# Grice-Lab/HmmUFOtu

Measured on AMD Instinct MI355X. Metric: reads placed/sec (whole node), gg_97_otus GTR+dGamma 250bp; HBM GB/s %peak, higher is better.
Workload: dtype f64; 1 GPU; gg_97_otus-scale synthetic DB (198643 nodes x 7682 CS columns, K=1400), GTR+dGamma(4), SE 250 bp amplicon reads, batch 8192 reads/step/GPU, 6 batches in flight, seeds in the reference's std::sort order (k_seed_refsort); seed_order=reference, message_window_cols=7682, parallelism=read-sharded x1

## Files before the change

### hmmufotu_amd/csrc/hu_engine.hip

```cpp
#include <algorithm>
#include <cmath>
#include <cstdio>
#include <cstring>
#include <limits>
#include <map>
#include <atomic>
#include <thread>
#include <memory>
#include <mutex>
#include <chrono>
#include <fstream>
#include <sstream>
#include <new>
#include <stdexcept>
#include "hu_common.h"
#include "hu_kern_sep.h"
#include "hu_kern_align.h"
#include "hu_kern_tree.h"
#include "hu_kern_blk.h"
#include "hu_kern_refsort.h"
#include "hu_kern_rank.h"
#include "hu_kern_anneal.h"
#include "hu_kern_build.h"
#include "hu_kern_otucs.h"
// ... 2267 lines not shown
		HIPCHK(hu_wait(b->stream));
	}
	b->seedCap = 1;
	for(size_t r = 0; r < n; ++r) b->seedCap = std::max(b->seedCap, (int) n_seeds[r]);
	b->state = ST_SEEDED;
	return HU_OK;
} catch(...) { return hu_catch_all("hu_seed_batch_given"); }

__global__ void k_seed_sortkeys(int n, const int32_t* __restrict__ seedCnt, const int32_t* __restrict__ seedId, uint32_t* __restrict__ key, uint32_t* __restrict__ val) {
	const int i = blockIdx.x * 256 + threadIdx.x;
	if(i >= n * HU_MAX_SEEDS) return;
	key[i] = (i % HU_MAX_SEEDS) < seedCnt[i / HU_MAX_SEEDS] ? (uint32_t) seedId[i] : 0xffffffffu;
	val[i] = (uint32_t) i;
}

static void plan_width_split(hu_batch* b) {
	b->rMain = 0; b->wideReads.clear(); b->maxAll = b->maxMain = 1;
	if((int) b->hStart.size() < b->n || (int) b->hEnd.size() < b->n) return;
	std::vector<int> R((size_t) b->n);
	for(int r = 0; r < b->n; ++r) { R[r] = std::max(0, b->hEnd[r] - b->hStart[r] + 1); b->maxAll = std::max(b->maxAll, R[r]); }
	b->maxMain = b->maxAll;
	if(!b->knob.width_split || b->n < 256) return;
	const int W = std::min(64, b->n / 128);
	std::vector<int> tmp(R);
	std::nth_element(tmp.begin(), tmp.begin() + W, tmp.end(), std::greater<int>());
	const int kth = tmp[W];
	static const int bounds[] = {512, 768, 1024, 1536, 2048, 3072};
	int bound = 0;
	for(int x : bounds) if(kth <= x) { bound = x; break; }
	if(!bound || bound >= b->maxAll) return;
	b->rMain = bound; b->maxMain = 1;
	for(int r = 0; r < b->n; ++r) { if(R[r] > bound) b->wideReads.push_back(r); else b->maxMain = std::max(b->maxMain, R[r]); }
	if(b->knob.trace) fprintf(stderr, "[hu] width split: %zu of %d reads beyond %d columns (widest %d) take a launch of their own\n", b->wideReads.size(), b->n, bound, b->maxAll);
}
static HuDbDev width_pass_dev(const hu_batch* b, int pass, const uint32_t* wideList) {
	HuDbDev dev = b->db->dev;
	if(b->rMain) { dev.rLo = pass ? b->rMain : -1; dev.rHi = pass ? 0x7fffffff : b->rMain; dev.wideList = pass ? wideList : nullptr; }
	return dev;
}

extern "C" int hu_estimate_batch(hu_batch* b, const hu_opts* o) try {
	if(!b || !o) return HU_ERR_ARG;
	if(b->state < ST_SEEDED) { hu_set_error("hu_estimate_batch: no seeds"); return HU_ERR_STATE; }
	HIPCHK(hipSetDevice(b->db->device));
	const size_t n = (size_t) b->n;
	int rc;
	if((rc = b->dEst.ensure(n * HU_MAX_SEEDS)) != HU_OK) return rc;
	(void) hipGetLastError();
	if(n) {
		Timer t(b, HU_T_ESTIMATE);
		plan_width_split(b);
		const bool stream = b->knob.streaming_sep != 0;
		if(b->rMain) {
			b->hWideOrd.clear();
			for(int r : b->wideReads) for(int sd = 0; sd < HU_MAX_SEEDS; ++sd) b->hWideOrd.push_back((uint32_t) r * HU_MAX_SEEDS + sd);
			if((rc = b->dWideOrd.ensure(b->hWideOrd.size())) != HU_OK) return rc;
			HIPCHK(hipMemcpyAsync(b->dWideOrd.p, b->hWideOrd.data(), b->hWideOrd.size() * 4, hipMemcpyHostToDevice, b->stream));
		}
		for(int pass = 0; pass < (b->rMain ? 2 : 1); ++pass) {
			const int maxR = pass ? b->maxAll : b->maxMain;
			const HuDbDev dev = width_pass_dev(b, pass, b->dWideOrd.p);
			#define EST_ARGS dev, b->db->mdl, b->dCodes.p, b->dStart.p, b->dEnd.p, b->dParDN.p, b->dSeedCnt.p, b->dSeedId.p, b->dSeedDN.p, o->weighted, b->dEst.p
			const unsigned eg = pass ? (unsigned) b->hWideOrd.size() : (unsigned) b->n * HU_MAX_SEEDS;
			const uint32_t* order = nullptr;
			if(pass) order = b->dWideOrd.p;
			else if(!b->knob.est_unsorted) {
				if((rc = b->dSortK.ensure((size_t) eg * 2)) != HU_OK || (rc = b->dSortV.ensure((size_t) eg * 2)) != HU_OK) return rc;
				k_seed_sortkeys<<<(eg + 255) / 256, 256, 0, b->stream>>>(b->n, b->dSeedCnt.p, b->dSeedId.p, b->dSortK.p, b->dSortV.p);
				if((rc = order_by_key(b, b->dSortK.p, b->dSortV.p, (size_t) eg, (uint32_t) b->db->dev.nNodes, b->dSortV.p + eg, false)) != HU_OK) return rc;
				order = b->dSortV.p + eg;
			}
			const int spt = (maxR + 255) / 256;
			const int xm = b->knob.xcd_map;
			const unsigned egl = pass ? eg : order ? std::min<unsigned>(eg, (unsigned) b->n * (unsigned) b->seedCap) : eg;
			const int var = b->knob.est_var;
			if(stream || spt > 12) k_estimate<<<eg, 64, 0, b->stream>>>(EST_ARGS);
			else if(var == 2) {
				if(spt <= 2) k_estimate_blk<2, 256><<<eg, 256, 0, b->stream>>>(EST_ARGS);
				else if(spt <= 4) k_estimate_blk<4, 256><<<eg, 256, 0, b->stream>>>(EST_ARGS);
				else if(spt <= 6) k_estimate_blk<6, 256><<<eg, 256, 0, b->stream>>>(EST_ARGS);
				else if(spt <= 8) k_estimate_blk<8, 256><<<eg, 256, 0, b->stream>>>(EST_ARGS);
				else k_estimate_blk<12, 256><<<eg, 256, 0, b->stream>>>(EST_ARGS);
			}
			else if(var == 1 && spt <= 6) k_estimate_prod<12, 2><<<egl, 128, 0, b->stream>>>(EST_ARGS, order, xm);
			else if(var == 3 && spt <= 6) k_estimate_prod<6, 4, 1><<<egl, 256, 0, b->stream>>>(EST_ARGS, order, xm);
			else if(spt <= 2) k_estimate_prod<2, 4><<<egl, 256, 0, b->stream>>>(EST_ARGS, order, xm);
			else if(spt <= 4) k_estimate_prod<4, 4><<<egl, 256, 0, b->stream>>>(EST_ARGS, order, xm);
			else if(spt <= 6) k_estimate_prod<6, 4, 4><<<egl, 256, (size_t)(b->knob.est_lds_pad > 0 && b->knob.est_lds_pad <= 60 ? b->knob.est_lds_pad : 0) * 1024, b->stream>>>(EST_ARGS, order, xm);
			else if(spt <= 8) k_estimate_prod<8, 4><<<egl, 256, 0, b->stream>>>(EST_ARGS, order, xm);
			else if(var == 4) k_estimate_prod<12, 4><<<egl, 256, 0, b->stream>>>(EST_ARGS, order, xm);
			else k_estimate_prod<6, 8, 2><<<egl, 512, 0, b->stream>>>(EST_ARGS, order, xm);
			#undef EST_ARGS
		}
	}
	HIPCHK(hipGetLastError());
	if(n) {
		if((rc = b->dPermCnt.ensure(n * 2)) != HU_OK) return rc;
		k_site_count<<<b->n, 64, 0, b->stream>>>(b->db->dev, b->n, b->dCodes.p, b->dStart.p, b->dEnd.p, b->dPermCnt.p);
		HIPCHK(hipGetLastError());
	}
	b->state = ST_ESTIMATED;
	return HU_OK;
} catch(...) { return hu_catch_all("hu_estimate_batch"); }


static int sync_host_cands(hu_batch* b) {
	if(b->hostCands) return HU_OK;
	const size_t n = (size_t) b->n;
	std::vector<int32_t> off(n + 1, 0);
	b->places.resize(b->nc);
	HIPCHK(hipSetDevice(b->db->device));
	if(n) HIPCHK(hipMemcpyAsync(off.data(), b->dCandOff.p, (n + 1) * 4, hipMemcpyDeviceToHost, b->stream));
	if(b->nc) HIPCHK(hipMemcpyAsync(b->places.data(), b->dPlaces.p, b->nc * sizeof(HuPlaceRec), hipMemcpyDeviceToHost, b->stream));
	HIPCHK(hu_wait(b->stream));
	b->candOffs.assign(off.begin(), off.end());
	b->hostCands = true;
	return HU_OK;
}
static int scan_cands(hu_batch* b, bool withPerm) {
	int rc;
	if((rc = b->dCandOff.ensure((size_t) b->n + 1)) != HU_OK || (rc = b->dMeta.ensure(4)) != HU_OK) return rc;
	k_cand_scan<<<1, 1024, 0, b->stream>>>(b->n, b->dCandCnt.p, b->dCandOff.p, withPerm ? b->dPermCnt.p : nullptr, b->dStart.p, b->dEnd.p, b->dMeta.p, b->rMain);
	HIPCHK(hipGetLastError());
	b->hMeta.assign(4, 0);
	int32_t* meta = b->hMeta.data();
	HIPCHK(hipMemcpyAsync(meta, b->dMeta.p, 12, hipMemcpyDeviceToHost, b->stream));
	if(b->rMain) { b->hCandOffAll.resize((size_t) b->n + 1); HIPCHK(hipMemcpyAsync(b->hCandOffAll.data(), b->dCandOff.p, ((size_t) b->n + 1) * 4, hipMemcpyDeviceToHost, b->stream)); }
	HIPCHK(hu_wait(b->stream));
	b->nc = (size_t) meta[0]; b->maxGapSites = meta[1]; b->maxBaseSites = meta[2];
	return HU_OK;
}

extern "C" int hu_filter_batch(hu_batch* b, const hu_opts* o) try {
	if(!b || !o) return HU_ERR_ARG;
	if(b->state < ST_ESTIMATED) { hu_set_error("hu_filter_batch: no estimates"); return HU_ERR_STATE; }
	if(!(o->max_error >= 0)) { hu_set_error("max_error must be >= 0"); return HU_ERR_ARG; }
	HIPCHK(hipSetDevice(b->db->device));
	const size_t n = (size_t) b->n;
	if(b->knob.inject_fault == 1) parallel_for(std::max<size_t>(n, 600), [&](size_t r) { if(r + 1 == std::max<size_t>(n, 600)) throw std::bad_alloc(); });
	int rc;
	if((rc = b->dCandCnt.ensure(std::max<size_t>(n, 1))) != HU_OK || (rc = b->dFiltSlot.ensure(std::max<size_t>(n, 1) * HU_MAX_SEEDS)) != HU_OK) return rc;
	(void) hipGetLastError();
	b->nc = 0; b->maxGapSites = b->maxBaseSites = 0;
	if(n) {
		k_filter<<<(unsigned)((n + 3) / 4), 256, 0, b->stream>>>(b->n, b->dSeedCnt.p, b->dEst.p, o->max_error, b->dCandCnt.p, b->dFiltSlot.p, b->knob.sort_seq);
		HIPCHK(hipGetLastError());
		if((rc = scan_cands(b, true)) != HU_OK) return rc;
		if((rc = b->dCands.ensure(std::max<size_t>(b->nc, 1))) != HU_OK || (rc = b->dPlaces.ensure(std::max<size_t>(b->nc, 1))) != HU_OK) return rc;
		k_build_cands<<<(unsigned)((n * HU_MAX_SEEDS + 255) / 256), 256, 0, b->stream>>>(b->db->dev, b->n, b->dCandCnt.p, b->dCandOff.p, b->dFiltSlot.p, b->dSeedId.p, b->dEst.p, b->dCands.p, b->dPlaces.p);
		HIPCHK(hipGetLastError());
	}
	b->hostCands = false; b->placesGiven = false;
	b->state = ST_FILTERED;
	return HU_OK;
} catch(...) { return hu_catch_all("hu_filter_batch"); }

extern "C" int hu_batch_set_candidates(hu_batch* b, const int64_t* offs, const hu_place_rec* recs, int placed) try {
	if(!b || !offs) { hu_set_error("hu_batch_set_candidates: null argument"); return HU_ERR_ARG; }
	if(b->state < ST_ALIGNED) { hu_set_error("hu_batch_set_candidates: reads are not aligned"); return HU_ERR_STATE; }
	const hu_db* db = b->db;
	const size_t n = (size_t) b->n;
	if(offs[0] != 0) { hu_set_error("hu_batch_set_candidates: offs[0] must be 0"); return HU_ERR_ARG; }
	for(size_t r = 0; r < n; ++r) {
		const int64_t k = offs[r + 1] - offs[r];
		if(k < 0 || k > HU_MAX_SEEDS || (k > 0 && (!recs || b->hAlns[r].status != HU_READ_OK || b->hEnd[r] < b->hStart[r]))) {
			hu_set_error("hu_batch_set_candidates: read %zu: %lld candidates (0..%d, none for a read that is not placed)", r, (long long) k, HU_MAX_SEEDS); return HU_ERR_ARG;
// ... 23 lines not shown
	}
	{
		int rc;
		if((rc = b->dCandCnt.ensure(std::max<size_t>(n, 1))) != HU_OK || (rc = b->dCands.ensure(std::max<size_t>(nc, 1))) != HU_OK ||
				(rc = b->dPlaces.ensure(std::max<size_t>(nc, 1))) != HU_OK || (rc = b->dPermCnt.ensure(std::max<size_t>(n, 1) * 2)) != HU_OK) return rc;
		(void) hipGetLastError();
		if(n) {
			HIPCHK(hipMemcpyAsync(b->dCandCnt.p, hCnt.data(), n * 4, hipMemcpyHostToDevice, b->stream));
			if(nc) {
				HIPCHK(hipMemcpyAsync(b->dCands.p, b->hCands.data(), nc * sizeof(HuCand), hipMemcpyHostToDevice, b->stream));
				HIPCHK(hipMemcpyAsync(b->dPlaces.p, b->places.data(), nc * sizeof(HuPlaceRec), hipMemcpyHostToDevice, b->stream));
			}
			k_site_count<<<b->n, 64, 0, b->stream>>>(db->dev, b->n, b->dCodes.p, b->dStart.p, b->dEnd.p, b->dPermCnt.p);
			HIPCHK(hipGetLastError());
			plan_width_split(b);
			if((rc = scan_cands(b, true)) != HU_OK) return rc;
		}
		else { b->nc = 0; b->maxGapSites = b->maxBaseSites = 0; }
	}
	b->hostCands = true;
	b->placesGiven = placed != 0;
	b->fixedRoot = false;
	b->state = placed ? ST_PLACED : ST_FILTERED;
	return HU_OK;
} catch(...) { return hu_catch_all("hu_batch_set_candidates"); }

__global__ void k_cand_sortkeys(int nc, const HuCand* __restrict__ cands, uint32_t* __restrict__ key, uint32_t* __restrict__ val) {
	const int i = blockIdx.x * 256 + threadIdx.x;
	if(i >= nc) return;
	key[i] = (uint32_t) cands[i].node; val[i] = (uint32_t) i;
}

extern "C" int hu_place_batch(hu_batch* b, const hu_opts* o) try {
	if(!b || !o) return HU_ERR_ARG;
	if(b->state < ST_FILTERED) { hu_set_error("hu_place_batch: candidates are not filtered"); return HU_ERR_STATE; }
	HIPCHK(hipSetDevice(b->db->device));
	const size_t nc = b->nc;
	int rc;
	if((rc = b->dPlaceOut.ensure(std::max<size_t>(nc, 1))) != HU_OK) return rc;
	(void) hipGetLastError();
	if(nc) {
		Timer t(b, HU_T_PLACE);
		int passes = 1;
		if(b->rMain) {
			b->hWideCand.clear();
			if(b->hCandOffAll.size() < (size_t) b->n + 1) { hu_set_error("hu_place_batch: candidate offsets of the wide reads are missing"); return HU_ERR_STATE; }
			for(int r : b->wideReads) for(int32_t c = b->hCandOffAll[r]; c < b->hCandOffAll[r + 1]; ++c) b->hWideCand.push_back((uint32_t) c);
			if(!b->hWideCand.empty()) {
				if((rc = b->dWideCand.ensure(b->hWideCand.size())) != HU_OK) return rc;
				HIPCHK(hipMemcpyAsync(b->dWideCand.p, b->hWideCand.data(), b->hWideCand.size() * 4, hipMemcpyHostToDevice, b->stream));
				passes = 2;
			}
		}
		for(int pass = 0; pass < passes; ++pass) {
			const int maxR = pass ? b->maxAll : b->maxMain;
			const HuDbDev dev = width_pass_dev(b, pass, b->dWideCand.p);
			const unsigned grid = pass ? (unsigned) b->hWideCand.size() : (unsigned) nc;
			const int spt2 = (maxR + 127) / 128, spt4 = (maxR + 255) / 256;
			const bool stream = b->knob.streaming_sep != 0 || spt4 > 12;
			#define PL_ARGS dev, b->db->mdl, b->dCodes.p, b->dStart.p, b->dEnd.p, b->dCands.p, b->dPlaceOut.p
			if(stream) {
				const size_t lds = (size_t)(3 * HU_MAX_DGK * 4 + HU_MAX_DGK * 5 * 4 + maxR) * sizeof(double);
				if(lds > 160 * 1024) { hu_set_error("alignment region of %d columns does not fit the placement kernel's LDS", maxR); return HU_ERR_ARG; }
				if(lds > 64 * 1024) HIPCHK(hipFuncSetAttribute((const void*) k_place, hipFuncAttributeMaxDynamicSharedMemorySize, (int) lds));
				k_place<<<grid, 64, lds, b->stream>>>(PL_ARGS);
			}
			else {
				const int var = b->knob.place_var;
				const int xm = b->knob.xcd_map;
				const uint32_t* order = nullptr;
				if(pass) order = b->dWideCand.p;
				else if(!b->knob.place_unsorted) {
					if((rc = b->dSortK.ensure(nc * 2)) != HU_OK || (rc = b->dSortV.ensure(nc * 2)) != HU_OK) return rc;
					k_cand_sortkeys<<<(unsigned)((nc + 255) / 256), 256, 0, b->stream>>>((int) nc, b->dCands.p, b->dSortK.p, b->dSortV.p);
					if((rc = order_by_key(b, b->dSortK.p, b->dSortV.p, nc, (uint32_t) b->db->dev.nNodes, b->dSortV.p + nc, false)) != HU_OK) return rc;
					order = b->dSortV.p + nc;
				}
				#define PL_GO(S, NW, E, R, O) k_place_blk<S, NW, E, R, O><<<grid, 64 * NW, 0, b->stream>>>(PL_ARGS, nullptr, order, nullptr, nullptr, xm)
				if((var == 99 || var == 98) && spt4 <= 6) {
					DBuf<long long> ddb;
					if((rc = ddb.ensure(nc * 12)) != HU_OK) return rc;
					long long* dd = ddb.p;
					HIPCHK(hipMemsetAsync(dd, 0, nc * 12 * sizeof(long long), b->stream));
					if(var == 99) k_place_blk<6, 4, 3, 0, 1, true><<<grid, 256, 0, b->stream>>>(PL_ARGS, dd);
					else k_place_blk<12, 2, 3, 0, 2, true, 1><<<grid, 128, 0, b->stream>>>(PL_ARGS, dd);
					std::vector<long long> hd(nc * 12);
					HIPCHK(hipMemcpyAsync(hd.data(), dd, nc * 12 * sizeof(long long), hipMemcpyDeviceToHost, b->stream));
					HIPCHK(hu_wait(b->stream));
					double acc[8] = {0}, ae[4] = {0};
					for(size_t c = 0; c < nc; ++c) { for(int i = 0; i < 8; ++i) acc[i] += (double) hd[c * 8 + i]; for(int i = 0; i < 4; ++i) ae[i] += (double) hd[nc * 8 + c * 4 + i]; }
					fprintf(stderr, "[place dbg] per candidate (s_memtime ticks): load %.0f tables %.0f sweeps %.0f em %.0f total %.0f | outer %.2f em steps %.2f\n",
							acc[0] / nc, acc[1] / nc, acc[2] / nc, acc[3] / nc, acc[4] / nc, acc[5] / nc, acc[6] / nc);
					fprintf(stderr, "[place dbg] inside the EM steps, per step: arithmetic %.0f wave reduction %.0f exchange between the waves %.0f tail %.0f\n",
							ae[0] / acc[6], ae[1] / acc[6], ae[2] / acc[6], ae[3] / acc[6]);
				}
				else if(var == 4 && spt4 <= 6) PL_GO(6, 4, 1, 0, 1);
				else if(var == 5 && spt4 <= 6) PL_GO(6, 4, 2, 1, 1);
				else if(var == 6 && spt2 <= 12) PL_GO(12, 2, 1, 0, 2);
				else if(spt2 <= 4) PL_GO(4, 2, 3, 0, 2);
				else if(spt2 <= 12 && !(var == 7)) {
					const int S = spt2 <= 8 ? 8 : 12, G = S - 2;
					const bool split = !pass && !b->knob.place_nosplit && b->maxGapSites <= G * 128 && b->maxBaseSites <= (S - G) * 128;
					if(b->knob.trace) fprintf(stderr, "[hu] place: %zu candidates, max region %d, %d sites per thread, %s, %s\n", nc, maxR, S, split ? "gap/base split slots" : "column order", "EM across both waves");
					if(split) {
						if((rc = b->dPerm.ensure((size_t) b->n * S * 128)) != HU_OK) return rc;
						k_site_perm<<<b->n, 64, 0, b->stream>>>(dev, b->n, b->dCodes.p, b->dStart.p, b->dEnd.p, G * 128, (S - G) * 128, b->dPerm.p);
						if(S == 8 && var != 6) k_place_blk<8, 2, 3, 0, 3, false, 3, 6><<<grid, 128, 3 * 8 * 128 * sizeof(double), b->stream>>>(PL_ARGS, nullptr, order, b->dPerm.p, b->dPermCnt.p, xm);
						else if(S == 8) k_place_blk<8, 2, 3, 0, 2, false, 0, 6><<<grid, 128, 0, b->stream>>>(PL_ARGS, nullptr, order, b->dPerm.p, b->dPermCnt.p, xm);
						else k_place_blk<12, 2, 3, 0, 2, false, 1, 10><<<grid, 128, (size_t)(b->knob.place_lds_pad > 0 && b->knob.place_lds_pad <= 44 ? b->knob.place_lds_pad : 0) * 1024, b->stream>>>(PL_ARGS, nullptr, order, b->dPerm.p, b->dPermCnt.p, xm);
					}
					else if(S == 8) PL_GO(8, 2, 3, 0, 2);
					else k_place_blk<12, 2, 3, 0, 2, false, 1><<<grid, 128, 0, b->stream>>>(PL_ARGS, nullptr, order, nullptr, nullptr, xm);
				}
				else if(var == 7 && spt2 <= 12) PL_GO(12, 2, 3, 0, 2);
				else if(spt4 <= 8) PL_GO(8, 4, 3, 0, 1);
				else if(var == 9) PL_GO(12, 4, 3, 0, 1);
				else k_place_blk<12, 4, 3, 0, 2, false, 1><<<grid, 256, 0, b->stream>>>(PL_ARGS, nullptr, order, nullptr, nullptr, xm);
				#undef PL_GO
			}
			#undef PL_ARGS
		}
		HIPCHK(hipGetLastError());
		if(o->fix_root_loglik) {
			if((rc = b->dRootLL.ensure(nc)) != HU_OK) return rc;
			k_root_loglik<<<(unsigned) nc, 64, 0, b->stream>>>(b->db->dev, b->db->mdl, b->dCodes.p, b->dStart.p, b->dEnd.p, b->dCands.p, b->dPlaceOut.p, (int) nc, b->dRootLL.p);
			HIPCHK(hipGetLastError());
		}
	}
	b->fixedRoot = o->fix_root_loglik != 0 && nc > 0;
	b->placesGiven = false;
	b->state = ST_PLACED;
	return HU_OK;
} catch(...) { return hu_catch_all("hu_place_batch"); }


static int hu_alleq_table(int device) {
	static std::mutex mu; static bool done[64] = {false};
	std::lock_guard<std::mutex> lk(mu);
	if(device < 0 || device >= 64) { hu_set_error("device %d out of range", device); return HU_ERR_ARG; }
	if(done[device]) return HU_OK;
	(void) hipGetLastError();
	k_alleq_init<<<1, 128>>>();
	HIPCHK(hipGetLastError());
	HIPCHK(hipDeviceSynchronize());
	done[device] = true;
	return HU_OK;
}

extern "C" int hu_finish_batch(hu_batch* b, const hu_opts* o) try {
	if(!b || !o) return HU_ERR_ARG;
	if(b->state < ST_PLACED) { hu_set_error("hu_finish_batch: candidates are not placed"); return HU_ERR_STATE; }
	const hu_db* db = b->db;
	const size_t n = (size_t) b->n;
	if(b->knob.inject_fault == 2) throw std::length_error("injected");
	HIPCHK(hipSetDevice(db->device));
	b->best.assign(n, hu_place_rec());
	int rc;
	if((rc = b->dBest.ensure(std::max<size_t>(n, 1))) != HU_OK) return rc;
	(void) hipGetLastError();
	if(n) {
		if((rc = hu_alleq_table(db->device)) != HU_OK) return rc;
		k_finish<<<(unsigned)((n + 63) / 64), 64, 0, b->stream>>>(db->dev, b->n, b->dStart.p, b->dEnd.p, b->dCandOff.p, b->dPlaces.p, b->dPlaceOut.p,
				b->fixedRoot ? b->dRootLL.p : nullptr, db->dLlTab, db->dAnnoId, o->max_height, o->only_ml, o->prior, b->placesGiven ? 1 : 0, b->dBest.p, b->knob.sort_seq);
		HIPCHK(hipGetLastError());
		HIPCHK(hipMemcpyAsync(b->best.data(), b->dBest.p, n * sizeof(hu_place_rec), hipMemcpyDeviceToHost, b->stream));
		HIPCHK(hu_wait(b->stream));
	}
	b->hostCands = false;
	b->state = ST_FINISHED;
	return HU_OK;
} catch(...) { return hu_catch_all("hu_finish_batch"); }

extern "C" int hu_assign_batch(hu_batch* b, const hu_opts* o) try {
	int rc;
// ... 807 lines not shown
```

### hmmufotu_amd/csrc/hu_kern_blk.h

```cpp
#pragma once
#include "hu_kern_sep.h"

#define HU_BLK_THREADS 256

__device__ inline void lds_wave_sync() { asm volatile("s_waitcnt lgkmcnt(0)" ::: "memory"); }
__device__ inline void lds_barrier() { asm volatile("s_waitcnt lgkmcnt(0)\n\ts_barrier" ::: "memory"); }

template<int NW = 4>
__device__ inline double block_sum(double v, double* red, int& phase) {
	v = wave_sum_uniform(v);
	double* r = red + (phase & 1) * NW;
	if((threadIdx.x & 63) == 0) r[threadIdx.x >> 6] = v;
	lds_barrier();
	double s = r[0];
#pragma unroll
	for(int w = 1; w < NW; ++w) s += r[w];
	phase ^= 1;
	return s;
}
template<int NW = 4>
__device__ inline long long block_sum_ll(long long v, long long* red, int& phase) {
	for(int m = 32; m > 0; m >>= 1) v += __shfl_xor(v, m);
	long long* r = red + (phase & 1) * NW;
	if((threadIdx.x & 63) == 0) r[threadIdx.x >> 6] = v;
// ... 43 lines not shown
			const int j = tid + THREADS * t;
			const int jj = j < n ? j : 0;
			load4(db.up + (sOff + jj) * 4, eU[t]); load4(db.down + (sOff + jj) * 4, eV[t]);
			bb[t] = cd[jj];
			if(j < n) ksum += (long long) db.upK[sOff + jj] + (long long) db.downK[sOff + jj];
		}
#pragma unroll
		for(int t = 0; t < SPT; ++t) {
			double c[4];
			conv_eig(mdl, Eu, eU[t], z[t]);
			conv_eig(mdl, Ev, eV[t], c);
			for(int i = 0; i < 4; ++i) z[t][i] *= c[i];
		}
	}
	int phase = 0;
	double dsum = 0, nsum = 0;
#pragma unroll
	for(int t = 0; t < SPT; ++t) {
		if(tid + THREADS * t >= n) continue;
		const int b = bb[t];
		const int b1 = argmax4_tied_lin(z[t]), b2 = b >= 0 ? b : piMax;
		if(!weighted) { if(b1 != b2) dsum += 1; }
		else {
			const double w1 = sel4(z[t], b1) / ((z[t][0] + z[t][2]) + (z[t][1] + z[t][3]));
			const double w2 = b >= 0 ? 1.0 : piw[b2];
			if(b1 != b2) dsum += w1 * w2;
			nsum += w1 * w2;
		}
	}
	dsum = block_sum<NW>(dsum, red, phase);
	double wnr;
	if(!weighted) wnr = dsum / (double) n;
	else { nsum = block_sum<NW>(nsum, red, phase); wnr = dsum / nsum; }
	double En[4], Ppi[4];
#pragma unroll
	for(int k = 0; k < 4; ++k) En[k] = exp(mdl.lam[k] * wnr);
	{ double a[4]; to_eig(mdl, mdl.pi, a); if(wnr == 0) { for(int i = 0; i < 4; ++i) Ppi[i] = mdl.pi[i]; } else conv_eig(mdl, En, a, Ppi); }
	double ll = 0;
#pragma unroll
	for(int t = 0; t < SPT; ++t) {
		if(tid + THREADS * t >= n) continue;
		const int b = bb[t];
		double c[4];
		if(b >= 0) {
			if(wnr == 0) { for(int i = 0; i < 4; ++i) c[i] = i == b ? 1.0 : 0.0; }
			else { double a[4]; for(int k = 0; k < 4; ++k) a[k] = mdl.U1[k*4+b]; conv_eig(mdl, En, a, c); }
		}
		else for(int i = 0; i < 4; ++i) c[i] = Ppi[i];
		ll += log((mdl.pi[0] * z[t][0] * c[0] + mdl.pi[2] * z[t][2] * c[2]) + (mdl.pi[1] * z[t][1] * c[1] + mdl.pi[3] * z[t][3] * c[3]));
	}
	ll = block_sum<NW>(ll, red, phase);
	int lphase = 0;
	const long long kt = block_sum_ll<NW>(ksum, redl, lphase);
	ll += (double) kt * HU_LN2;
	if(tid == 0) { HuEstOut o; o.ratio = ratio; o.wnr = wnr; o.loglik = ll; out[(size_t) read * HU_MAX_SEEDS + s] = o; }
}

template<int CTRL>
__device__ inline double dpp_mul_full(double v) {
	const int lo = __builtin_amdgcn_mov_dpp(__double2loint(v), CTRL, 0xf, 0xf, true);
	const int hi = __builtin_amdgcn_mov_dpp(__double2hiint(v), CTRL, 0xf, 0xf, true);
	return v * __hiloint2double(hi, lo);
}
__device__ inline double wave_prod(double v) {
	v = dpp_mul_full<0xB1>(v);
	v = dpp_mul_full<0x4E>(v);
	v = dpp_mul_full<0x141>(v);
	v = dpp_mul_full<0x140>(v);
	v *= __shfl_xor(v, 16);
	v *= __shfl_xor(v, 32);
	return v;
}
__device__ inline int wave_sum_i32(int v) {
	for(int m = 32; m > 0; m >>= 1) v += __shfl_xor(v, m);
	return v;
}

__device__ inline uint32_t hu_xcd_pos(uint32_t b, uint32_t nb, int xmap) {
	if(!xmap) return b;
	const uint32_t per = nb >> 3;
	return b < per * 8 ? (b & 7u) * per + (b >> 3) : b;
}

template<int SPT, int NW, int OCC = 1>
__global__ __launch_bounds__(64 * NW, OCC) void k_estimate_prod(HuDbDev db, HuModelDev mdl, const int8_t* __restrict__ codes,
		const int32_t* __restrict__ rstart, const int32_t* __restrict__ rend, const uint32_t* __restrict__ parDN,
		const int32_t* __restrict__ seedCnt, const int32_t* __restrict__ seedId, const uint32_t* __restrict__ seedDN,
		int weighted, HuEstOut* __restrict__ out, const uint32_t* __restrict__ order, int xmap = 0) {
	constexpr int THREADS = 64 * NW;
	__shared__ double redd[2 * NW];
	__shared__ int redi[2 * NW];
	__shared__ __attribute__((aligned(16))) double Qtab[NW][24];
	const uint32_t slot = order ? order[hu_xcd_pos(blockIdx.x, gridDim.x, xmap)] : blockIdx.x;
	const int read = slot / HU_MAX_SEEDS, s = slot % HU_MAX_SEEDS, tid = threadIdx.x, lane = tid & 63, wave = tid >> 6;
	if(s >= seedCnt[read] || hu_skip_width(db, rend[read] - rstart[read] + 1)) return;
	const int un = seedId[(size_t) read * HU_MAX_SEEDS + s];
	const int vn = db.parent[un];
	const uint32_t dn = seedDN[(size_t) read * HU_MAX_SEEDS + s];
	const uint32_t pv = parDN[(size_t) read * HU_MAX_SEEDS + s];
	const double cDist = (double)(dn >> 16) / (double)(dn & 0xffffu);
	const double pDist = (double)(pv >> 16) / (double)(pv & 0xffffu);
	double ratio = cDist / (cDist + pDist);
	if(isnan(ratio)) ratio = 0.5;
	const double w0 = db.blen[un];
	const double wur = w0 * ratio, wvr = w0 - wur;
	double Eu[3], Ev[3];
	{
		const int l6 = lane < 6 ? lane : 0, m3 = l6 % 3;
		const double e = exp((m3 == 0 ? mdl.lam[1] : m3 == 1 ? mdl.lam[2] : mdl.lam[3]) * (l6 < 3 ? wur : wvr));
		const int lo = __double2loint(e), hi = __double2hiint(e);
#pragma unroll
		for(int k = 0; k < 3; ++k) {
			Eu[k] = __hiloint2double(__builtin_amdgcn_readlane(hi, k), __builtin_amdgcn_readlane(lo, k));
			Ev[k] = __hiloint2double(__builtin_amdgcn_readlane(hi, 3 + k), __builtin_amdgcn_readlane(lo, 3 + k));
		}
	}
	const int start = rstart[read], end = rend[read], n = end - start + 1;
	const int8_t* __restrict__ cd = codes + (size_t) read * db.csLen + start;
	const int64_t sOff = (int64_t) un * db.winLen + (start - db.winStart);
	const int piMax = argmax4d(mdl.logpi);
	double z[SPT][4]; unsigned long long bop = 0; int ksum = 0;
	{
		double aU[SPT][4], aV[SPT][4];
#pragma unroll
		for(int t = 0; t < SPT; ++t) {
			const int j = tid + THREADS * t;
			const int jj = j < n ? j : 0;
			load4(db.up + (sOff + jj) * 4, aU[t]); load4(db.down + (sOff + jj) * 4, aV[t]);
			const int b = cd[jj];
			bop |= (unsigned long long)(b >= 0 ? b : 4) << (3 * t);
			if(j < n) ksum += db.upK[sOff + jj] + db.downK[sOff + jj];
		}
#pragma unroll
		for(int t = 0; t < SPT; ++t) {
			const double su1 = Eu[0] * aU[t][1], su2 = Eu[1] * aU[t][2], su3 = Eu[2] * aU[t][3];
			const double sv1 = Ev[0] * aV[t][1], sv2 = Ev[1] * aV[t][2], sv3 = Ev[2] * aV[t][3];
#pragma unroll
			for(int i = 0; i < 4; ++i) {
				const double cu = fmax(fma(mdl.U[i*4+3], su3, fma(mdl.U[i*4+2], su2, fma(mdl.U[i*4+1], su1, aU[t][0]))), 0.0);
				const double cv = fmax(fma(mdl.U[i*4+3], sv3, fma(mdl.U[i*4+2], sv2, fma(mdl.U[i*4+1], sv1, aV[t][0]))), 0.0);
				z[t][i] = cu * cv;
			}
		}
	}
	double wnr;
	if(!weighted) {
		int nd = 0;
#pragma unroll
		for(int t = 0; t < SPT; ++t) {
			const int bi = (int)((bop >> (3 * t)) & 7u);
			const int b1 = argmax4_tied_lin(z[t]), b2 = bi < 4 ? bi : piMax;
			nd += __popcll(__ballot(tid + THREADS * t < n && b1 != b2));
		}
		if(lane == 0) redi[wave] = nd;
		lds_barrier();
		int tot = redi[0];
#pragma unroll
		for(int w = 1; w < NW; ++w) tot += redi[w];
		wnr = (double) tot / (double) n;
	}
	else {
		double piw[4];
		{ double mx = max4d(mdl.logpi), sm; for(int i = 0; i < 4; ++i) piw[i] = exp(mdl.logpi[i] - mx); sm = (piw[0] + piw[2]) + (piw[1] + piw[3]); for(int i = 0; i < 4; ++i) piw[i] /= sm; }
		double dsum = 0, nsum = 0;
#pragma unroll
		for(int t = 0; t < SPT; ++t) {
			if(tid + THREADS * t >= n) continue;
			const int bi = (int)((bop >> (3 * t)) & 7u);
			const int b1 = argmax4_tied_lin(z[t]), b2 = bi < 4 ? bi : piMax;
			const double w1 = sel4(z[t], b1) / ((z[t][0] + z[t][2]) + (z[t][1] + z[t][3]));
			const double w2 = bi < 4 ? 1.0 : piw[b2];
			if(b1 != b2) dsum += w1 * w2;
			nsum += w1 * w2;
		}
		dsum = wave_sum(dsum); nsum = wave_sum(nsum);
		if(lane == 0) { redd[wave] = dsum; redd[NW + wave] = nsum; }
		lds_barrier();
		double a = redd[0], c = redd[NW];
#pragma unroll
		for(int w = 1; w < NW; ++w) { a += redd[w]; c += redd[NW + w]; }
		wnr = a / c;
		lds_barrier();
	}
	double* Q = Qtab[wave];
	if(lane < 3) Q[1 + lane] = exp((lane == 0 ? mdl.lam[1] : lane == 1 ? mdl.lam[2] : mdl.lam[3]) * wnr);
	lds_wave_sync();
	if(lane < 20) {
		const int b = lane >> 2, i = lane & 3;
		const double pii = sel4(mdl.pi, i);
		double c;
		if(wnr == 0) c = b < 4 ? (i == b ? 1.0 : 0.0) : pii;
		else {
			double a0, a1, a2, a3;
			if(b < 4) { a0 = sel4(mdl.U1 + 0, b); a1 = sel4(mdl.U1 + 4, b); a2 = sel4(mdl.U1 + 8, b); a3 = sel4(mdl.U1 + 12, b); }
			else {
				a0 = (mdl.U1[0] * mdl.pi[0] + mdl.U1[1] * mdl.pi[1]) + (mdl.U1[2] * mdl.pi[2] + mdl.U1[3] * mdl.pi[3]);
				a1 = (mdl.U1[4] * mdl.pi[0] + mdl.U1[5] * mdl.pi[1]) + (mdl.U1[6] * mdl.pi[2] + mdl.U1[7] * mdl.pi[3]);
				a2 = (mdl.U1[8] * mdl.pi[0] + mdl.U1[9] * mdl.pi[1]) + (mdl.U1[10] * mdl.pi[2] + mdl.U1[11] * mdl.pi[3]);
				a3 = (mdl.U1[12] * mdl.pi[0] + mdl.U1[13] * mdl.pi[1]) + (mdl.U1[14] * mdl.pi[2] + mdl.U1[15] * mdl.pi[3]);
			}
			const double Ui1 = i == 0 ? mdl.U[1] : i == 1 ? mdl.U[5] : i == 2 ? mdl.U[9] : mdl.U[13];
			const double Ui2 = i == 0 ? mdl.U[2] : i == 1 ? mdl.U[6] : i == 2 ? mdl.U[10] : mdl.U[14];
			const double Ui3 = i == 0 ? mdl.U[3] : i == 1 ? mdl.U[7] : i == 2 ? mdl.U[11] : mdl.U[15];
			c = fmax(fma(Ui3, Q[3] * a3, fma(Ui2, Q[2] * a2, fma(Ui1, Q[1] * a1, a0))), 0.0);
		}
		Q[4 + b * 4 + i] = pii * c;
	}
	lds_wave_sync();
	double mant = 1.0; int esum = ksum;
#pragma unroll
	for(int t = 0; t < SPT; ++t) {
		const double* q = Q + 4 + ((bop >> (3 * t)) & 7u) * 4;
		double x = fmax(fma(q[3], z[t][3], fma(q[2], z[t][2], fma(q[1], z[t][1], q[0] * z[t][0]))), 0.0);
		if(tid + THREADS * t >= n) x = 1.0;
		mant *= __builtin_amdgcn_frexp_mant(x);
		esum += x == 0.0 ? 0 : __builtin_amdgcn_frexp_exp(x);
	}
	esum += __builtin_amdgcn_frexp_exp(mant); mant = __builtin_amdgcn_frexp_mant(mant);
	mant = wave_prod(mant);
	esum = wave_sum_i32(esum);
	if(lane == 0) { redd[wave] = mant; redi[NW + wave] = esum; }
	lds_barrier();
	if(tid == 0) {
		double m = redd[0]; long long e = redi[NW];
#pragma unroll
		for(int w = 1; w < NW; ++w) { m *= redd[w]; e += redi[NW + w]; }
		HuEstOut o; o.ratio = ratio; o.wnr = wnr; o.loglik = log(m) + (double) e * HU_LN2;
		out[(size_t) read * HU_MAX_SEEDS + s] = o;
	}
}

#define HU_RHO_SKIP 1e60
#define HU_TP 18
#define HU_EXP_MEPS 0.99999000004999983333
#define HU_EXP_PEPS 1.00001000005000016667

__device__ inline double fast_div(double a, double b) {
	double y = __builtin_amdgcn_rcp(b);
	y = fma(fma(-b, y, 1.0), y, y);
	y = fma(fma(-b, y, 1.0), y, y);
	const double q = a * y;
	return fma(fma(-b, q, a), y, q);
}

__device__ __attribute__((noinline)) double hu_exp_call(double x) { return exp(x); }
__device__ __attribute__((noinline)) double hu_log_call(double x) { return log(x); }

template<int SPT, int NW, int EMV, int RED>
__device__ inline double em_branch_blk(const double (&rho)[SPT], int nvalidWave, double w0, double maxL,
		double* red, double* redc, int& phase, int& emIters, long long* st = nullptr) {
	long long tl = st ? (long long) __builtin_amdgcn_s_memtime() : 0;
	auto stamp = [&](int i) { if(st) { const long long t = (long long) __builtin_amdgcn_s_memtime(); st[i] += t - tl; tl = t; } };
	const int lane = threadIdx.x & 63, wave = threadIdx.x >> 6;
	double q0 = hu_exp_call(-w0), p0 = 1 - q0, p = p0, q = q0, rc = 0;
	if(lane == 0) redc[(phase & 1) * NW + wave] = (double) nvalidWave;
	for(int it = 0; it < HU_MAX_ITER && p >= 0 && p <= 1; ++it) {
		double s = 0;
		const bool fast = q0 >= 1e-30 && p0 >= 1e-30;
		if(fast) {
			if(EMV == 3 && SPT % 4 == 0) {
				constexpr int G = SPT / 4;
				double x[SPT], ab[G], cd[G], X[G], nm[G], y[G], w[G];
#pragma unroll
				for(int t = 0; t < SPT; ++t) x[t] = fma(rho[t], q0, p0);
				__builtin_amdgcn_sched_barrier(0);
#pragma unroll
				for(int g = 0; g < G; ++g) { ab[g] = x[4 * g] * x[4 * g + 1]; cd[g] = x[4 * g + 2] * x[4 * g + 3]; }
#pragma unroll
				for(int g = 0; g < G; ++g) { X[g] = ab[g] * cd[g]; x[4 * g] += x[4 * g + 1]; x[4 * g + 2] += x[4 * g + 3]; }
				__builtin_amdgcn_sched_barrier(0);
#pragma unroll
				for(int g = 0; g < G; ++g) { y[g] = __builtin_amdgcn_rcp(X[g]); nm[g] = x[4 * g + 2] * ab[g]; }
#pragma unroll
				for(int g = 0; g < G; ++g) nm[g] = fma(x[4 * g], cd[g], nm[g]);
				__builtin_amdgcn_sched_barrier(0);
#pragma unroll
				for(int g = 0; g < G; ++g) { w[g] = fma(-X[g], y[g], 2.0); nm[g] *= y[g]; }
				__builtin_amdgcn_sched_barrier(0);
#pragma unroll
				for(int g = 0; g < G; ++g) s = fma(nm[g], w[g], s);
			}
			else if(EMV == 4 && SPT % 2 == 0) {
#pragma unroll
				for(int t = 0; t < SPT; t += 2) {
					const double a = fma(rho[t], q0, p0), bb = fma(rho[t + 1], q0, p0);
					const double x = a * bb, y = __builtin_amdgcn_rcp(x);
					s = fma((a + bb) * y, fma(-x, y, 2.0), s);
				}
			}
			else {
#pragma unroll
				for(int t = 0; t < SPT; ++t) {
					const double x = fma(rho[t], q0, p0);
					const double y = __builtin_amdgcn_rcp(x);
					if(EMV == 1 || EMV == 3 || EMV == 4) s = fma(y, fma(-x, y, 2.0), s);
					else { const double y1 = fma(fma(-x, y, 1.0), y, y); s = fma(y1, fma(-x, y1, 2.0), s); }
				}
			}
		}
		else {
#pragma unroll
			for(int t = 0; t < SPT; ++t) {
				const double r = rho[t];
				const double tt = p0 / fma(r, q0, p0);
				s += r == HU_RHO_SKIP ? 0.0 : tt;
			}
		}
		if(st) { if(s == 1.2345e-300) st[7] = 1; }
		stamp(0);
		s = wave_sum_uniform(s);
		stamp(1);
// ... 12 lines not shown
		}
		phase ^= 1;
		if(st) { if(s == 1.2345e-300) st[7] = 1; }
		stamp(2);
		if(fast) s *= p0;
		p = s * rc; q = 1 - p;
		++emIters;
		if(q0 * HU_EXP_MEPS < q && q < q0 * HU_EXP_PEPS) { stamp(3); break; }
		p0 = p; q0 = q;
		stamp(3);
	}
	double w = -hu_log_call(q);
	if(w > maxL) w = maxL;
	return w;
}

__global__ __launch_bounds__(64) void k_site_count(HuDbDev db, int n, const int8_t* __restrict__ codes, const int32_t* __restrict__ rstart,
		const int32_t* __restrict__ rend, int32_t* __restrict__ cnt) {
	const int read = blockIdx.x, lane = threadIdx.x;
	const int start = rstart[read], len = rend[read] - start + 1;
	int g = 0, bc = 0;
	for(int j0 = 0; j0 < len; j0 += 64) {
		const int j = j0 + lane;
		const bool val = j < len;
		const int b = val ? codes[(size_t) read * db.csLen + start + j] : 0;
		g += __popcll(__ballot(val && b < 0)); bc += __popcll(__ballot(val && b >= 0));
	}
	if(lane == 0) { cnt[2 * read] = g; cnt[2 * read + 1] = bc; }
}
__global__ __launch_bounds__(64) void k_site_perm(HuDbDev db, int n, const int8_t* __restrict__ codes, const int32_t* __restrict__ rstart,
		const int32_t* __restrict__ rend, int gapCap, int baseCap, uint16_t* __restrict__ perm) {
	const int read = blockIdx.x, lane = threadIdx.x;
	const int start = rstart[read], len = rend[read] - start + 1;
	if(hu_skip_width(db, len)) return;
	uint16_t* __restrict__ pr = perm + (size_t) read * (gapCap + baseCap);
	const unsigned long long lt = (1ull << lane) - 1ull;
	int g = 0, bc = 0;
	for(int j0 = 0; j0 < len; j0 += 64) {
		const int j = j0 + lane;
		const bool val = j < len;
		const int b = val ? codes[(size_t) read * db.csLen + start + j] : 0;
		const unsigned long long mg = __ballot(val && b < 0), mb = __ballot(val && b >= 0);
		if(val && b < 0) { const int at = g + __popcll(mg & lt); if(at < gapCap) pr[at] = (uint16_t) j; }
		if(val && b >= 0) { const int at = bc + __popcll(mb & lt); if(at < baseCap) pr[gapCap + at] = (uint16_t) j; }
		g += __popcll(mg); bc += __popcll(mb);
	}
}

template<int SPT, int NW, int EMV, int RED, int OCC, bool DBG = false, int VL = 0, int GS = 0>
__global__ __launch_bounds__(64 * NW, OCC) void k_place_blk(HuDbDev db, HuModelDev mdl, const int8_t* __restrict__ codes,
		const int32_t* __restrict__ rstart, const int32_t* __restrict__ rend,
		const HuCand* __restrict__ cands, HuPlaceOut* __restrict__ out, long long* __restrict__ dbg = nullptr, const uint32_t* __restrict__ order = nullptr,
		const uint16_t* __restrict__ perm = nullptr, const int32_t* __restrict__ permCnt = nullptr, int xmap = 0) {
	constexpr int THREADS = 64 * NW;
	long long tk[8] = {0, 0, 0, 0, 0, 0, 0, 0}, t0 = 0, tl = 0;
	long long te[8] = {0, 0, 0, 0, 0, 0, 0, 0};
	auto stamp = [&](int slot) { if(DBG) { const long long t = (long long) __builtin_amdgcn_s_memtime(); tk[slot] += t - tl; tl = t; } };
	if(DBG) { t0 = tl = (long long) __builtin_amdgcn_s_memtime(); }
	__shared__ double red[2 * NW], redc[2 * NW];
	__shared__ double cst[HU_PC_COUNT];
	__shared__ double Etab[3 * HU_MAX_DGK * 4];
	__shared__ double Gtab[16];
	__shared__ __attribute__((aligned(16))) double tabM[5 * HU_TP];
	__shared__ __attribute__((aligned(16))) double tabD[6 * 4];
	__shared__ double vl[VL == 1 ? SPT * 64 * NW : 1];
	extern __shared__ double vdyn[];
	const int tid = threadIdx.x;
	const int vt = (tid + 64 * (blockIdx.x % NW)) % THREADS;
	const uint32_t ci = order ? order[hu_xcd_pos(blockIdx.x, gridDim.x, xmap)] : blockIdx.x;
	const HuCand cd = cands[ci];
	const int read = cd.read, un = cd.node;
	const int start = rstart[read], end = rend[read], n = end - start + 1;
	if(hu_skip_width(db, n)) return;
	const int Kc = mdl.dgK > 0 ? mdl.dgK : 1;
	const double rKc = 1.0 / (double) Kc;
	const int8_t* __restrict__ cdr = codes + (size_t) read * db.csLen + start;
	const int64_t mOff = ((int64_t) un * db.winLen + (start - db.winStart)) * 4;
	const double* __restrict__ Ub = db.up + mOff;
	const double* __restrict__ Vb = db.down + mOff;
	const int nGap = GS > 0 ? permCnt[2 * read] : 0, nBase = GS > 0 ? permCnt[2 * read + 1] : 0;
	double u[SPT][3], v[SPT][3]; unsigned long long bop = 0, bop2 = 0;
	{
		double aU[SPT][4], aV[SPT][4];
#pragma unroll
		for(int t = 0; t < SPT; ++t) {
			int jj;
			if(GS > 0) {
				const int i = t < GS ? tid + THREADS * t : tid + THREADS * (t - GS);
				const bool val = i < (t < GS ? nGap : nBase);
				jj = val ? (int) perm[(size_t) read * (SPT * THREADS) + (t < GS ? 0 : GS * THREADS) + i] : 0;
			}
			else { const int j = tid + THREADS * t; jj = j < n ? j : 0; }
			load4(Ub + (size_t) jj * 4, aU[t]); load4(Vb + (size_t) jj * 4, aV[t]);
			const int b = cdr[jj];
			if(t < 21) bop |= (unsigned long long)(b >= 0 ? b : 4) << (3 * t);
			else bop2 |= (unsigned long long)(b >= 0 ? b : 4) << (3 * (t - 21));
		}
#pragma unroll
		for(int t = 0; t < SPT; ++t) {
			const double iu = 1.0 / aU[t][0], iv = 1.0 / aV[t][0];
#pragma unroll
			for(int m = 0; m < 3; ++m) { u[t][m] = aU[t][m + 1] * iu; v[t][m] = aV[t][m + 1] * iv; }
			if(VL == 1) { vl[t * THREADS + tid] = v[t][2]; v[t][2] = 0; }
			if(VL == 3) {
#pragma unroll
				for(int m = 0; m < 3; ++m) { vdyn[(m * SPT + t) * THREADS + tid] = v[t][m]; v[t][m] = 0; }
			}
		}
	}
	for(int i = tid; i < HU_PC_COUNT; i += THREADS) cst[i] = db.placeConst[i];
	lds_barrier();
	const double* clam = cst + HU_PC_LAM; const double* crate = cst + HU_PC_RATE; const double* cW = cst + HU_PC_W;
	const double* cC = cst + HU_PC_C; const double* ccb = cst + HU_PC_CB;
	const double w0 = db.blen[un];
	double lenUR = w0 * cd.ratio0, lenVR = w0 * (1 - cd.ratio0), lenNR = cd.wnr0;
	double wur0 = lenUR, wnr0 = lenNR;
	const double w0j = lenUR + lenVR;
	double wur = wur0, wnr = wnr0;
	int iter = 0, emIters = 0, phase = 0;
	double rho[SPT];
	if(DBG) { double x = 0; for(int t = 0; t < SPT; ++t) x += u[t][0] + u[t][1]; if(x == 1.2345e-300) tk[7] = 1; }
	stamp(0);
	for(; iter < HU_MAX_ITER && 0 <= wur && wur <= w0j; ++iter) {
		if(vt < 8 * Kc) {
			const int which = vt / (4 * Kc), k = (vt >> 2) % Kc, m = vt & 3;
			Etab[(which * HU_MAX_DGK + k) * 4 + m] = hu_exp_call(clam[m] * ((which ? lenVR : lenUR) * crate[k]));
		}
		lds_barrier();
		if(vt < 16) {
			const int m = vt >> 2, nn = vt & 3;
			double g = 0;
			for(int k = 0; k < Kc; ++k) g += Etab[k * 4 + m] * Etab[(HU_MAX_DGK + k) * 4 + nn];
			Gtab[vt] = g * rKc;
		}
		lds_barrier();
		for(int e = vt; e < 84; e += THREADS) {
			if(e < 80) tabM[(e >> 4) * HU_TP + (e & 15)] = cW[e] * Gtab[e & 15];
			else tabD[e - 80] = Gtab[(e - 80) * 5];
		}
		lds_barrier();
		stamp(1);
		int nv = 0;
		{
			unsigned long long bq = bop, bq2 = bop2;
			asm volatile("" : "+v"(bq), "+v"(bq2));
			const double g0 = tabD[0], g1 = tabD[1], g2 = tabD[2], g3 = tabD[3];
			double Mg[GS > 0 ? 16 : 1];
			if(GS > 0) {
#pragma unroll
				for(int e = 0; e < 16; ++e) Mg[e] = tabM[4 * HU_TP + e];
			}
#pragma unroll
			for(int t = 0; t < SPT; ++t) {
				const double* M = (GS > 0 && t < GS) ? Mg : tabM + (unsigned)(((t < 21 ? bq >> (3 * t) : bq2 >> (3 * (t - 21)))) & 7u) * HU_TP;
				const double v0 = VL == 3 ? vdyn[(0 * SPT + t) * THREADS + tid] : v[t][0], v1 = VL == 3 ? vdyn[(1 * SPT + t) * THREADS + tid] : v[t][1];
				const double v2 = VL == 3 ? vdyn[(2 * SPT + t) * THREADS + tid] : VL == 1 ? vl[t * THREADS + tid] : v[t][2];
				double num = fma(M[3], v2, fma(M[2], v1, fma(M[1], v0, M[0])));
#pragma unroll
				for(int m = 1; m < 4; ++m) {
					const double tm = fma(M[m * 4 + 3], v2, fma(M[m * 4 + 2], v1, fma(M[m * 4 + 1], v0, M[m * 4 + 0])));
					num = fma(tm, u[t][m - 1], num);
				}
				const double den = fma(g3 * u[t][2], v2, fma(g2 * u[t][1], v1, fma(g1 * u[t][0], v0, g0)));
				const double r = fast_div(num, den);
				const bool inr = GS > 0 ? (t < GS ? tid + THREADS * t < nGap : tid + THREADS * (t - GS) < nBase) : tid + THREADS * t < n;
				const bool ok = inr && fabs(r) < HU_RHO_SKIP;
				rho[t] = ok ? r : HU_RHO_SKIP;
				nv += __popcll(__ballot(ok));
			}
		}
		stamp(2);
		wnr = em_branch_blk<SPT, NW, EMV, RED>(rho, nv, lenNR, 1.0, red, redc, phase, emIters, DBG ? te : nullptr);
		lenNR = wnr;
		stamp(3);
		if(vt < 4 * Kc) {
			const int k = vt >> 2, m = vt & 3;
			Etab[(2 * HU_MAX_DGK + k) * 4 + m] = hu_exp_call(clam[m] * (lenNR * crate[k]));
		}
		lds_barrier();
		if(vt < 16) {
// ... 67 lines not shown
```

Baseline: 380,100 reads/s.

## Batch estimate/place loads ahead of use and raise estimate kernel occupancy bounds

The estimate kernel now issues all upK/downK scaling loads first, then all up/down message loads, separated by scheduling barriers, and folds the scaling sums afterward. This aims to keep more memory requests in flight instead of interleaving dependent loads. The place kernel likewise gathers all permuted site indices before issuing the message loads. Launch bounds for the estimate kernel now request more waves per SIMD depending on sites per thread, which may cap registers and cause spills. Timing-instrumented debug variants (var 98) are added for both kernels.

```diff
diff --git a/hmmufotu_amd/csrc/hu_engine.hip b/hmmufotu_amd/csrc/hu_engine.hip
--- a/hmmufotu_amd/csrc/hu_engine.hip
+++ b/hmmufotu_amd/csrc/hu_engine.hip
@@ -2373,6 +2373,18 @@
 				else if(spt <= 8) k_estimate_blk<8, 256><<<eg, 256, 0, b->stream>>>(EST_ARGS);
 				else k_estimate_blk<12, 256><<<eg, 256, 0, b->stream>>>(EST_ARGS);
 			}
+			else if(var == 98 && spt > 4 && spt <= 6) {
+				DBuf<long long> ddb;
+				if((rc = ddb.ensure((size_t) egl * 4)) != HU_OK) return rc;
+				HIPCHK(hipMemsetAsync(ddb.p, 0, (size_t) egl * 4 * sizeof(long long), b->stream));
+				k_estimate_prod<6, 4, 4, true><<<egl, 256, 0, b->stream>>>(EST_ARGS, order, xm, ddb.p);
+				std::vector<long long> hd((size_t) egl * 4);
+				HIPCHK(hipMemcpyAsync(hd.data(), ddb.p, hd.size() * sizeof(long long), hipMemcpyDeviceToHost, b->stream));
+				HIPCHK(hu_wait(b->stream));
+				double acc[4] = {0}; size_t ran = 0;
+				for(size_t c = 0; c < (size_t) egl; ++c) if(hd[c * 4 + 3]) { ++ran; for(int i = 0; i < 4; ++i) acc[i] += (double) hd[c * 4 + i]; }
+				if(ran) fprintf(stderr, "[est dbg] per slot (s_memtime ticks, %zu slots): prologue %.0f load %.0f rest %.0f total %.0f\n", ran, acc[0] / ran, acc[1] / ran, acc[2] / ran, acc[3] / ran);
+			}
 			else if(var == 1 && spt <= 6) k_estimate_prod<12, 2><<<egl, 128, 0, b->stream>>>(EST_ARGS, order, xm);
 			else if(var == 3 && spt <= 6) k_estimate_prod<6, 4, 1><<<egl, 256, 0, b->stream>>>(EST_ARGS, order, xm);
 			else if(spt <= 2) k_estimate_prod<2, 4><<<egl, 256, 0, b->stream>>>(EST_ARGS, order, xm);
@@ -2562,14 +2574,21 @@
 					if((rc = ddb.ensure(nc * 12)) != HU_OK) return rc;
 					long long* dd = ddb.p;
 					HIPCHK(hipMemsetAsync(dd, 0, nc * 12 * sizeof(long long), b->stream));
+					const bool split98 = var == 98 && !pass && !b->knob.place_nosplit && spt2 > 8 && b->maxGapSites <= 10 * 128 && b->maxBaseSites <= 2 * 128;
 					if(var == 99) k_place_blk<6, 4, 3, 0, 1, true><<<grid, 256, 0, b->stream>>>(PL_ARGS, dd);
-					else k_place_blk<12, 2, 3, 0, 2, true, 1><<<grid, 128, 0, b->stream>>>(PL_ARGS, dd);
+					else if(split98) {
+						if((rc = b->dPerm.ensure((size_t) b->n * 12 * 128)) != HU_OK) return rc;
+						k_site_perm<<<b->n, 64, 0, b->stream>>>(dev, b->n, b->dCodes.p, b->dStart.p, b->dEnd.p, 10 * 128, 2 * 128, b->dPerm.p);
+						k_place_blk<12, 2, 3, 0, 2, true, 1, 10><<<grid, 128, 0, b->stream>>>(PL_ARGS, dd, order, b->dPerm.p, b->dPermCnt.p, xm);
+					}
+					else k_place_blk<12, 2, 3, 0, 2, true, 1><<<grid, 128, 0, b->stream>>>(PL_ARGS, dd, order, nullptr, nullptr, xm);
 					std::vector<long long> hd(nc * 12);
 					HIPCHK(hipMemcpyAsync(hd.data(), dd, nc * 12 * sizeof(long long), hipMemcpyDeviceToHost, b->stream));
 					HIPCHK(hu_wait(b->stream));
 					double acc[8] = {0}, ae[4] = {0};
 					for(size_t c = 0; c < nc; ++c) { for(int i = 0; i < 8; ++i) acc[i] += (double) hd[c * 8 + i]; for(int i = 0; i < 4; ++i) ae[i] += (double) hd[nc * 8 + c * 4 + i]; }
-					fprintf(stderr, "[place dbg] per candidate (s_memtime ticks): load %.0f tables %.0f sweeps %.0f em %.0f total %.0f | outer %.2f em steps %.2f\n",
+					fprintf(stderr, "[place dbg] %s, per candidate (s_memtime ticks): load %.0f tables %.0f sweeps %.0f em %.0f total %.0f | outer %.2f em steps %.2f\n",
+							var == 99 ? "4 waves x 6 sites" : split98 ? "2 waves x 12 sites, gap/base split slots" : "2 waves x 12 sites, column order",
 							acc[0] / nc, acc[1] / nc, acc[2] / nc, acc[3] / nc, acc[4] / nc, acc[5] / nc, acc[6] / nc);
 					fprintf(stderr, "[place dbg] inside the EM steps, per step: arithmetic %.0f wave reduction %.0f exchange between the waves %.0f tail %.0f\n",
 							ae[0] / acc[6], ae[1] / acc[6], ae[2] / acc[6], ae[3] / acc[6]);
diff --git a/hmmufotu_amd/csrc/hu_kern_blk.h b/hmmufotu_amd/csrc/hu_kern_blk.h
--- a/hmmufotu_amd/csrc/hu_kern_blk.h
+++ b/hmmufotu_amd/csrc/hu_kern_blk.h
@@ -149,12 +149,19 @@
 	return b < per * 8 ? (b & 7u) * per + (b >> 3) : b;
 }
 
-template<int SPT, int NW, int OCC = 1>
-__global__ __launch_bounds__(64 * NW, OCC) void k_estimate_prod(HuDbDev db, HuModelDev mdl, const int8_t* __restrict__ codes,
+__host__ __device__ constexpr int hu_est_waves(int spt, int occ) {
+	const int w = spt <= 2 ? 8 : spt <= 4 ? 5 : spt <= 6 ? 4 : spt <= 8 ? 3 : 2;
+	return occ > w ? occ : w;
+}
+template<int SPT, int NW, int OCC = 1, bool DBG = false>
+__global__ __launch_bounds__(64 * NW, hu_est_waves(SPT, OCC)) void k_estimate_prod(HuDbDev db, HuModelDev mdl, const int8_t* __restrict__ codes,
 		const int32_t* __restrict__ rstart, const int32_t* __restrict__ rend, const uint32_t* __restrict__ parDN,
 		const int32_t* __restrict__ seedCnt, const int32_t* __restrict__ seedId, const uint32_t* __restrict__ seedDN,
-		int weighted, HuEstOut* __restrict__ out, const uint32_t* __restrict__ order, int xmap = 0) {
+		int weighted, HuEstOut* __restrict__ out, const uint32_t* __restrict__ order, int xmap = 0, long long* __restrict__ dbg = nullptr) {
 	constexpr int THREADS = 64 * NW;
+	long long tk[4] = {0, 0, 0, 0}, t0 = 0, tl = 0;
+	auto stamp = [&](int i) { if(DBG) { const long long t = (long long) __builtin_amdgcn_s_memtime(); tk[i] += t - tl; tl = t; } };
+	if(DBG) { t0 = tl = (long long) __builtin_amdgcn_s_memtime(); }
 	__shared__ double redd[2 * NW];
 	__shared__ int redi[2 * NW];
 	__shared__ __attribute__((aligned(16))) double Qtab[NW][24];
@@ -187,17 +194,36 @@
 	const int64_t sOff = (int64_t) un * db.winLen + (start - db.winStart);
 	const int piMax = argmax4d(mdl.logpi);
 	double z[SPT][4]; unsigned long long bop = 0; int ksum = 0;
+	double aU[SPT][4], aV[SPT][4];
+	const double* __restrict__ Ub = db.up + sOff * 4; const double* __restrict__ Vb = db.down + sOff * 4;
+	const int32_t* __restrict__ upKb = db.upK + sOff; const int32_t* __restrict__ downKb = db.downK + sOff;
+	auto inr = [&](int t) { return tid < n - THREADS * t; };
+	stamp(0);
 	{
-		double aU[SPT][4], aV[SPT][4];
-#pragma unroll
-		for(int t = 0; t < SPT; ++t) {
-			const int j = tid + THREADS * t;
-			const int jj = j < n ? j : 0;
-			load4(db.up + (sOff + jj) * 4, aU[t]); load4(db.down + (sOff + jj) * 4, aV[t]);
+		int kU[SPT], kV[SPT];
+#pragma unroll
+		for(int t = 0; t < SPT; ++t) {
+			const int jj = inr(t) ? tid + THREADS * t : 0;
+			kU[t] = upKb[(size_t) jj]; kV[t] = downKb[(size_t) jj];
+		}
+		__builtin_amdgcn_sched_barrier(0);
+#pragma unroll
+		for(int t = 0; t < SPT; ++t) {
+			const int jj = inr(t) ? tid + THREADS * t : 0;
+			load4(Ub + (size_t) jj * 4, aU[t]); load4(Vb + (size_t) jj * 4, aV[t]);
 			const int b = cd[jj];
 			bop |= (unsigned long long)(b >= 0 ? b : 4) << (3 * t);
-			if(j < n) ksum += db.upK[sOff + jj] + db.downK[sOff + jj];
-		}
+		}
+		__builtin_amdgcn_sched_barrier(0);
+#pragma unroll
+		for(int t = 0; t < SPT; ++t) {
+			asm volatile("" : "+v"(kU[t]), "+v"(kV[t]));
+			ksum += inr(t) ? kU[t] + kV[t] : 0;
+		}
+	}
+	if(DBG) { double x = 0; for(int t = 0; t < SPT; ++t) x += aU[t][0] + aV[t][0]; if(x == 1.2345e-300 || bop == ~0ull) tk[2] = 1; }
+	stamp(1);
+	{
 #pragma unroll
 		for(int t = 0; t < SPT; ++t) {
 			const double su1 = Eu[0] * aU[t][1], su2 = Eu[1] * aU[t][2], su3 = Eu[2] * aU[t][3];
@@ -217,7 +243,7 @@
 		for(int t = 0; t < SPT; ++t) {
 			const int bi = (int)((bop >> (3 * t)) & 7u);
 			const int b1 = argmax4_tied_lin(z[t]), b2 = bi < 4 ? bi : piMax;
-			nd += __popcll(__ballot(tid + THREADS * t < n && b1 != b2));
+			nd += __popcll(__ballot(inr(t) && b1 != b2));
 		}
 		if(lane == 0) redi[wave] = nd;
 		lds_barrier();
@@ -232,7 +258,7 @@
 		double dsum = 0, nsum = 0;
 #pragma unroll
 		for(int t = 0; t < SPT; ++t) {
-			if(tid + THREADS * t >= n) continue;
+			if(!inr(t)) continue;
 			const int bi = (int)((bop >> (3 * t)) & 7u);
 			const int b1 = argmax4_tied_lin(z[t]), b2 = bi < 4 ? bi : piMax;
 			const double w1 = sel4(z[t], b1) / ((z[t][0] + z[t][2]) + (z[t][1] + z[t][3]));
@@ -279,7 +305,7 @@
 	for(int t = 0; t < SPT; ++t) {
 		const double* q = Q + 4 + ((bop >> (3 * t)) & 7u) * 4;
 		double x = fmax(fma(q[3], z[t][3], fma(q[2], z[t][2], fma(q[1], z[t][1], q[0] * z[t][0]))), 0.0);
-		if(tid + THREADS * t >= n) x = 1.0;
+		if(!inr(t)) x = 1.0;
 		mant *= __builtin_amdgcn_frexp_mant(x);
 		esum += x == 0.0 ? 0 : __builtin_amdgcn_frexp_exp(x);
 	}
@@ -294,6 +320,10 @@
 		for(int w = 1; w < NW; ++w) { m *= redd[w]; e += redi[NW + w]; }
 		HuEstOut o; o.ratio = ratio; o.wnr = wnr; o.loglik = log(m) + (double) e * HU_LN2;
 		out[(size_t) read * HU_MAX_SEEDS + s] = o;
+	}
+	if(DBG) {
+		stamp(2);
+		if(tid == 0) { tk[3] = tl - t0; for(int i = 0; i < 4; ++i) dbg[(size_t) blockIdx.x * 4 + i] = tk[i]; }
 	}
 }
 
@@ -472,20 +502,26 @@
 	double u[SPT][3], v[SPT][3]; unsigned long long bop = 0, bop2 = 0;
 	{
 		double aU[SPT][4], aV[SPT][4];
-#pragma unroll
-		for(int t = 0; t < SPT; ++t) {
-			int jj;
+		int js[SPT];
+#pragma unroll
+		for(int t = 0; t < SPT; ++t) {
 			if(GS > 0) {
 				const int i = t < GS ? tid + THREADS * t : tid + THREADS * (t - GS);
 				const bool val = i < (t < GS ? nGap : nBase);
-				jj = val ? (int) perm[(size_t) read * (SPT * THREADS) + (t < GS ? 0 : GS * THREADS) + i] : 0;
-			}
-			else { const int j = tid + THREADS * t; jj = j < n ? j : 0; }
+				const int e = (int) perm[(size_t) read * (SPT * THREADS) + (t < GS ? 0 : GS * THREADS) + (val ? i : 0)];
+				js[t] = val ? e : 0;
+			}
+			else { const int j = tid + THREADS * t; js[t] = j < n ? j : 0; }
+		}
+#pragma unroll
+		for(int t = 0; t < SPT; ++t) {
+			const int jj = js[t];
 			load4(Ub + (size_t) jj * 4, aU[t]); load4(Vb + (size_t) jj * 4, aV[t]);
 			const int b = cdr[jj];
 			if(t < 21) bop |= (unsigned long long)(b >= 0 ? b : 4) << (3 * t);
 			else bop2 |= (unsigned long long)(b >= 0 ? b : 4) << (3 * (t - 21));
 		}
+		__builtin_amdgcn_sched_barrier(0);
 #pragma unroll
 		for(int t = 0; t < SPT; ++t) {
 			const double iu = 1.0 / aU[t][0], iv = 1.0 / aV[t][0];
```

Result: faster. 397,000 reads/s, median of 6 (+4.4%).
